# quan-dao/practical-collab-perception

Hardware: AMD Instinct MI355X
Metric: frames/sec (60k-pt cloud, 6 agents) (higher is better)
Workload: dtype f32

## Files before the change

practical-collab-perception_amd/csrc/sparseconv.hip:

```cpp
#include "pcp_common.h"

namespace {

constexpr int SP_TH = 8, SP_TW = 16, SP_PIX = SP_TH * SP_TW;
constexpr int SP_CIN = 64;
constexpr int SP_ALD = 68;
constexpr int SP_THREADS = 256;

struct SpParams {
  const float *pf;
  const int *cell_rank;
  const float *w;
  const float *bias;
  float *out;
  int batch, nx, ny, ho, wo, ld_out, cout, relu;
  int tiles_x, tiles_y;
};


template <bool OUT_BF16>
__global__ __launch_bounds__(SP_THREADS, 2) void k_sparse_conv_s2(SpParams p) {
  __shared__ __attribute__((aligned(16))) float acc[SP_PIX * 64];
#ifdef SP_ROW_SPLIT
  __shared__ __attribute__((aligned(16))) float atile[2][32 * SP_ALD];
#else
  __shared__ __attribute__((aligned(16))) float atile[4][32 * SP_ALD];
#endif
  __shared__ int row_rank[9][SP_PIX];
  __shared__ unsigned char row_pix[9][SP_PIX];
  __shared__ int cnt[9][2];

  const int tid = threadIdx.x, lane = tid & 63;
  const int wave = __builtin_amdgcn_readfirstlane(tid >> 6);
  int sp = blockIdx.x;
  const int tile_x = sp % p.tiles_x;
  sp /= p.tiles_x;
  const int tile_y = sp % p.tiles_y;
  const int b = sp / p.tiles_y;
  const int oy0 = tile_y * SP_TH, ox0 = tile_x * SP_TW;
  const int plane = p.nx * p.ny;

  int rank[9];
  {
    const int py = tid >> 4, px = tid & 15;
    const int oy = oy0 + py, ox = ox0 + px;
    const bool pix_ok = tid < SP_PIX && oy < p.ho && ox < p.wo;
#pragma unroll
    for (int t = 0; t < 9; t++) {
      const int iy = 2 * oy + t / 3 - 1, ix = 2 * ox + t % 3 - 1;
      rank[t] = -1;
      if (pix_ok && iy >= 0 && iy < p.ny && ix >= 0 && ix < p.nx) rank[t] = p.cell_rank[(long long)b * plane + ix * p.ny + iy];
    }
  }
  for (int i = tid; i < SP_PIX * 64; i += SP_THREADS) acc[i] = 0.f;
  int pre[9];
#pragma unroll
  for (int t = 0; t < 9; t++) {
    const unsigned long long bal = __ballot(rank[t] >= 0);
    pre[t] = __popcll(bal & ((1ULL << lane) - 1ULL));
    if (lane == 0 && wave < 2) cnt[t][wave] = __popcll(bal);
  }
  __syncthreads();
  int total = 0;
#pragma unroll
  for (int t = 0; t < 9; t++) {
    const int c0 = cnt[t][0], c1 = cnt[t][1];
    total += c0 + c1;
    if (tid < SP_PIX && rank[t] >= 0) {
      const int row = (wave == 1 ? c0 : 0) + pre[t];
      row_rank[t][row] = rank[t];
      row_pix[t][row] = (unsigned char)tid;
    }
  }
  __syncthreads();

#ifdef SP_ROW_SPLIT
  if (total > 0) {
    const int rh = wave >> 1, nh = wave & 1;
    const int m16 = lane & 15, q4 = lane >> 4;
    const int g_row = tid >> 3, g_q = (tid & 7) * 2;
    __shared__ unsigned char item_tap[36], item_chunk[36];
    __shared__ int n_items_s;
    if (tid == 0) {
      int k = 0;
      for (int t = 0; t < 9; t++)
        for (int c0 = 0; c0 < cnt[t][0] + cnt[t][1]; c0 += 32) { item_tap[k] = (unsigned char)t; item_chunk[k] = (unsigned char)(c0 >> 5); k++; }
      n_items_s = k;
    }
    __syncthreads();
    const int n_items = n_items_s;
    constexpr int DEPTH = 4;
    f32x4 g[DEPTH][2];
    f32x4 wq[2][2][4];
    auto gather = [&](int k, f32x4 (&dst)[2]) {
      const int kc = min(k, n_items - 1);
      const int t = item_tap[kc], c0 = item_chunk[kc] * 32;
      const int row = min(c0 + g_row, cnt[t][0] + cnt[t][1] - 1);
      const float *src = p.pf + (long long)row_rank[t][row] * SP_CIN + g_q * 4;
      dst[0] = *reinterpret_cast<const f32x4 *>(src);
      dst[1] = *reinterpret_cast<const f32x4 *>(src + 4);
    };
    auto wload = [&](int k, f32x4 (&dst)[2][4]) {
      const int t = item_tap[min(k, n_items - 1)];
#pragma unroll
      for (int s2 = 0; s2 < 2; s2++) {
        const float *wr = p.w + ((long long)(t * 64 + nh * 32 + s2 * 16 + m16)) * SP_CIN + 4 * q4;
#pragma unroll
        for (int j = 0; j < 4; j++) dst[s2][j] = *reinterpret_cast<const f32x4 *>(wr + 16 * j);
      }
    };
    wload(0, wq[0]);
    __builtin_amdgcn_sched_barrier(0);
    wload(1, wq[1]);
    __builtin_amdgcn_sched_barrier(0);
#pragma unroll
    for (int u = 0; u < DEPTH; u++) {
      gather(u, g[u]);
      __builtin_amdgcn_sched_barrier(0);
    }
    auto stage = [&](int k, f32x4 (&gu)[2], f32x4 (&wu)[2][4], float *at) {
          const int t = item_tap[k], c0 = item_chunk[k] * 32;
      const int rows = min(32, cnt[t][0] + cnt[t][1] - c0);
      const bool live = g_row < rows;
      const f32x4 zero4 = f32x4{0.f, 0.f, 0.f, 0.f};
      *reinterpret_cast<f32x4 *>(at + g_row * SP_ALD + g_q * 4) = live ? gu[0] : zero4;
      *reinterpret_cast<f32x4 *>(at + g_row * SP_ALD + g_q * 4 + 4) = live ? gu[1] : zero4;
      __builtin_amdgcn_sched_barrier(0);
      gather(k + DEPTH, gu);
      __builtin_amdgcn_sched_barrier(0);
      const unsigned pix4 = *reinterpret_cast<const unsigned *>(&row_pix[t][min(c0 + rh * 16 + q4 * 4, SP_PIX - 4)]);
      __syncthreads();
      typedef float f32x4c __attribute__((ext_vector_type(4)));
      f32x4c c0v = {0.f, 0.f, 0.f, 0.f}, c1v = {0.f, 0.f, 0.f, 0.f};
      const float *xa = at + (rh * 16 + m16) * SP_ALD + 4 * q4;
      f32x4 a[4];
#pragma unroll
      for (int j = 0; j < 4; j++) a[j] = *reinterpret_cast<const f32x4 *>(xa + 16 * j);
      int pixs[4];
      float old0[4], old1[4];
      const int col = nh * 32 + m16;
#pragma unroll
      for (int i = 0; i < 4; i++) {
        const int row = rh * 16 + q4 * 4 + i;
        pixs[i] = row < rows ? (int)((pix4 >> (8 * i)) & 255u) : -1;
        const int pa = pixs[i] >= 0 ? pixs[i] : 0;
        old0[i] = acc[pa * 64 + col];
        old1[i] = acc[pa * 64 + col + 16];
      }
#pragma unroll
      for (int j = 0; j < 4; j++)
#pragma unroll
        for (int kk = 0; kk < 4; kk++) {
          c0v = __builtin_amdgcn_mfma_f32_16x16x4f32(a[j][kk], wu[0][j][kk], c0v, 0, 0, 0);
          c1v = __builtin_amdgcn_mfma_f32_16x16x4f32(a[j][kk], wu[1][j][kk], c1v, 0, 0, 0);
        }
      __builtin_amdgcn_sched_barrier(0);
      wload(k + 2, wu);
      __builtin_amdgcn_sched_barrier(0);
#pragma unroll
      for (int i = 0; i < 4; i++)
        if (pixs[i] >= 0) {
          acc[pixs[i] * 64 + col] = old0[i] + c0v[i];
          acc[pixs[i] * 64 + col + 16] = old1[i] + c1v[i];
        }
    };
    int k0 = 0;
    for (; k0 + DEPTH <= n_items; k0 += DEPTH) {
      stage(k0 + 0, g[0], wq[0], atile[0]);
      stage(k0 + 1, g[1], wq[1], atile[1]);
      stage(k0 + 2, g[2], wq[0], atile[0]);
      stage(k0 + 3, g[3], wq[1], atile[1]);
    }
    if (k0 + 0 < n_items) stage(k0 + 0, g[0], wq[0], atile[0]);
    if (k0 + 1 < n_items) stage(k0 + 1, g[1], wq[1], atile[1]);
    if (k0 + 2 < n_items) stage(k0 + 2, g[2], wq[0], atile[0]);
    __syncthreads();
  }

#else
  if (total > 0) {
    const int m16 = lane & 15, q4 = lane >> 4;
    const int g_row = tid >> 3, g_q = (tid & 7) * 2;
    __shared__ unsigned char item_tap[36], item_chunk[36];
    __shared__ int n_items_s;
    if (tid == 0) {
      int k = 0;
      for (int t = 0; t < 9; t++)
        for (int c0 = 0; c0 < cnt[t][0] + cnt[t][1]; c0 += 32) { item_tap[k] = (unsigned char)t; item_chunk[k] = (unsigned char)(c0 >> 5); k++; }
      n_items_s = k;
    }
    __syncthreads();
    const int n_items = n_items_s;
    f32x4 g[4][2];
    f32x4 wq[4][4];
    auto gather = [&](int k, f32x4 (&dst)[2]) {
      const int kc = min(k, n_items - 1);
      const int t = item_tap[kc], c0 = item_chunk[kc] * 32;
      const int row = min(c0 + g_row, cnt[t][0] + cnt[t][1] - 1);
      const float *src = p.pf + (long long)row_rank[t][row] * SP_CIN + g_q * 4;
      dst[0] = *reinterpret_cast<const f32x4 *>(src);
      dst[1] = *reinterpret_cast<const f32x4 *>(src + 4);
    };
    auto wload = [&](int k, f32x4 (&dst)[4]) {
      const int t = item_tap[min(k, n_items - 1)];
      const float *wr = p.w + ((long long)(t * 64 + wave * 16 + m16)) * SP_CIN + 4 * q4;
#pragma unroll
      for (int j = 0; j < 4; j++) dst[j] = *reinterpret_cast<const f32x4 *>(wr + 16 * j);
    };
#pragma unroll
    for (int u = 0; u < 4; u++) {
      wload(u, wq[u]);
      gather(u, g[u]);
      __builtin_amdgcn_sched_barrier(0);
    }
    typedef float f32x4c __attribute__((ext_vector_type(4)));
    const int col = wave * 16 + m16;
    auto stage = [&](int k, f32x4 (&g0)[2], f32x4 (&g1)[2], f32x4 (&w0)[4], f32x4 (&w1)[4], float *at0, float *at1) {
      const f32x4 zero4 = f32x4{0.f, 0.f, 0.f, 0.f};
      int rows_i[2], tap_i[2], c0_i[2];
#pragma unroll
      for (int it = 0; it < 2; it++) {
        const int kk = min(k + it, n_items - 1);
        tap_i[it] = item_tap[kk];
        c0_i[it] = item_chunk[kk] * 32;
        rows_i[it] = (k + it < n_items) ? min(32, cnt[tap_i[it]][0] + cnt[tap_i[it]][1] - c0_i[it]) : 0;
      }
      *reinterpret_cast<f32x4 *>(at0 + g_row * SP_ALD + g_q * 4) = g_row < rows_i[0] ? g0[0] : zero4;
      *reinterpret_cast<f32x4 *>(at0 + g_row * SP_ALD + g_q * 4 + 4) = g_row < rows_i[0] ? g0[1] : zero4;
      *reinterpret_cast<f32x4 *>(at1 + g_row * SP_ALD + g_q * 4) = g_row < rows_i[1] ? g1[0] : zero4;
      *reinterpret_cast<f32x4 *>(at1 + g_row * SP_ALD + g_q * 4 + 4) = g_row < rows_i[1] ? g1[1] : zero4;
      __builtin_amdgcn_sched_barrier(0);
      gather(k + 4, g0);
      gather(k + 5, g1);
      __builtin_amdgcn_sched_barrier(0);
      unsigned pix4[2][2];
#pragma unroll
      for (int it = 0; it < 2; it++)
#pragma unroll
        for (int rtile = 0; rtile < 2; rtile++)
          pix4[it][rtile] = *reinterpret_cast<const unsigned *>(&row_pix[tap_i[it]][min(c0_i[it] + rtile * 16 + q4 * 4, SP_PIX - 4)]);
      __syncthreads();
      int pixs[2][2][4];
      float old0[2][4];
#pragma unroll
      for (int it = 0; it < 2; it++)
#pragma unroll
        for (int rtile = 0; rtile < 2; rtile++)
#pragma unroll
          for (int i = 0; i < 4; i++)
            pixs[it][rtile][i] = (rtile * 16 + q4 * 4 + i < rows_i[it]) ? (int)((pix4[it][rtile] >> (8 * i)) & 255u) : -1;
#pragma unroll
      for (int rtile = 0; rtile < 2; rtile++)
#pragma unroll
        for (int i = 0; i < 4; i++) old0[rtile][i] = acc[max(pixs[0][rtile][i], 0) * 64 + col];
      f32x4c cv[2][2];
#pragma unroll
      for (int it = 0; it < 2; it++) {
        const float *at = it == 0 ? at0 : at1;
#pragma unroll
        for (int rtile = 0; rtile < 2; rtile++) {
          f32x4c c = {0.f, 0.f, 0.f, 0.f};
          if (rows_i[it] > 16 * rtile) {
            f32x4 a[4];
#pragma unroll
            for (int j = 0; j < 4; j++) a[j] = *reinterpret_cast<const f32x4 *>(at + (rtile * 16 + m16) * SP_ALD + 16 * j + 4 * q4);
#pragma unroll
            for (int j = 0; j < 4; j++)
#pragma unroll
              for (int kk = 0; kk < 4; kk++) c = __builtin_amdgcn_mfma_f32_16x16x4f32(a[j][kk], (it == 0 ? w0 : w1)[j][kk], c, 0, 0, 0);
          }
          cv[it][rtile] = c;
        }
      }
      __builtin_amdgcn_sched_barrier(0);
      wload(k + 4, w0);
      wload(k + 5, w1);
      __builtin_amdgcn_sched_barrier(0);
#pragma unroll
      for (int rtile = 0; rtile < 2; rtile++)
#pragma unroll
        for (int i = 0; i < 4; i++)
          if (pixs[0][rtile][i] >= 0) acc[pixs[0][rtile][i] * 64 + col] = old0[rtile][i] + cv[0][rtile][i];
      float old1[2][4];
#pragma unroll
      for (int rtile = 0; rtile < 2; rtile++)
#pragma unroll
        for (int i = 0; i < 4; i++) old1[rtile][i] = acc[max(pixs[1][rtile][i], 0) * 64 + col];
#pragma unroll
      for (int rtile = 0; rtile < 2; rtile++)
#pragma unroll
        for (int i = 0; i < 4; i++)
          if (pixs[1][rtile][i] >= 0) acc[pixs[1][rtile][i] * 64 + col] = old1[rtile][i] + cv[1][rtile][i];
    };
    int k0 = 0;
    for (; k0 + 4 <= n_items; k0 += 4) {
      stage(k0 + 0, g[0], g[1], wq[0], wq[1], atile[0], atile[1]);
      stage(k0 + 2, g[2], g[3], wq[2], wq[3], atile[2], atile[3]);
    }
    if (k0 + 0 < n_items) stage(k0 + 0, g[0], g[1], wq[0], wq[1], atile[0], atile[1]);
    if (k0 + 2 < n_items) stage(k0 + 2, g[2], g[3], wq[2], wq[3], atile[2], atile[3]);
    __syncthreads();
  }
#endif

  {
    const int n4 = (tid & 15) * 4;
    const f32x4 bv = *reinterpret_cast<const f32x4 *>(p.bias + n4);
#pragma unroll
    for (int i = 0; i < 8; i++) {
      const int pix = (tid >> 4) + 16 * i;
      const int oy = oy0 + (pix >> 4), ox = ox0 + (pix & 15);
      if (oy < p.ho && ox < p.wo && n4 < p.cout) {
        f32x4 v = *reinterpret_cast<const f32x4 *>(acc + pix * 64 + n4) + bv;
        if (p.relu) {
          v.x = fmaxf(v.x, 0.f);
          v.y = fmaxf(v.y, 0.f);
          v.z = fmaxf(v.z, 0.f);
          v.w = fmaxf(v.w, 0.f);
        }
        const long long o = ((long long)(b * p.ho + oy) * p.wo + ox) * p.ld_out + n4;
        if (OUT_BF16) {
          typedef __bf16 b4 __attribute__((ext_vector_type(4)));
          b4 q;
          q[0] = (__bf16)v.x; q[1] = (__bf16)v.y; q[2] = (__bf16)v.z; q[3] = (__bf16)v.w;
          *reinterpret_cast<b4 *>(reinterpret_cast<__bf16 *>(p.out) + o) = q;
        } else {
          *reinterpret_cast<f32x4 *>(p.out + o) = v;
        }
      }
    }
  }
}

}

static int sparse_conv_impl(const float *pillar_features, const pcp_grid_t *grid, const void *vox_workspace, int64_t n, const float *w_packed,
                            const float *bias, int32_t cout, int32_t relu, void *out, int out_bf16, int32_t ld_out, void *stream_) {
  if (!pillar_features || !grid || !vox_workspace || !w_packed || !bias || !out || n < 0) return PCP_ERR_ARG;
  if (cout <= 0 || cout > 64 || cout % 4 != 0 || ld_out % 4 != 0 || ld_out < cout) return PCP_ERR_UNSUPPORTED;
  if ((((uintptr_t)pillar_features) & 15) || (((uintptr_t)w_packed) & 15) || (((uintptr_t)bias) & 15) || (((uintptr_t)out) & (out_bf16 ? 7 : 15)))
    return PCP_ERR_ARG;
  if (grid->batch_size <= 0 || grid->nx <= 0 || grid->ny <= 0) return PCP_ERR_ARG;
  const int64_t cells = (int64_t)grid->batch_size * grid->nx * grid->ny;
  VoxLayout L = pcp_vox_layout(cells, n);
  SpParams p;
  p.pf = pillar_features;
  p.cell_rank = reinterpret_cast<const int *>(reinterpret_cast<const char *>(vox_workspace) + L.cell_rank);
  p.w = w_packed; p.bias = bias; p.out = (float *)out;
  p.batch = grid->batch_size; p.nx = grid->nx; p.ny = grid->ny;
  p.ho = (grid->ny - 1) / 2 + 1;
  p.wo = (grid->nx - 1) / 2 + 1;
  p.ld_out = ld_out; p.cout = cout; p.relu = relu;
  p.tiles_x = (p.wo + SP_TW - 1) / SP_TW;
  p.tiles_y = (p.ho + SP_TH - 1) / SP_TH;
  const long long blocks = (long long)p.batch * p.tiles_x * p.tiles_y;
  if (blocks > 0x7fffffffLL) return PCP_ERR_ARG;
  if (out_bf16) hipLaunchKernelGGL(k_sparse_conv_s2<true>, dim3((unsigned)blocks), dim3(SP_THREADS), 0, (hipStream_t)stream_, p);
  else hipLaunchKernelGGL(k_sparse_conv_s2<false>, dim3((unsigned)blocks), dim3(SP_THREADS), 0, (hipStream_t)stream_, p);
  PCP_CHECK_LAUNCH();
  return PCP_OK;
}

extern "C" int pcp_sparse_conv3x3_s2(const float *pillar_features, const pcp_grid_t *grid, const void *vox_workspace, int64_t n,
                                     const float *w_packed, const float *bias, int32_t cout, int32_t relu, float *out, int32_t ld_out,
                                     void *stream_) {
  return sparse_conv_impl(pillar_features, grid, vox_workspace, n, w_packed, bias, cout, relu, out, 0, ld_out, stream_);
}

extern "C" int pcp_mp_sparse_conv3x3_s2(const float *pillar_features, const pcp_grid_t *grid, const void *vox_workspace, int64_t n,
                                        const float *w_packed, const float *bias, int32_t cout, int32_t relu, void *out, int32_t out_dtype,
                                        int32_t ld_out, void *stream_) {
  if (out_dtype != 0 && out_dtype != 1) return PCP_ERR_ARG;
  return sparse_conv_impl(pillar_features, grid, vox_workspace, n, w_packed, bias, cout, relu, out, out_dtype, ld_out, stream_);
}
```

Before: 398.7.

## Make sparse conv kernel persistent with cross-tile prefetch of ranks and features

Turns the sparse 3x3 stride-2 conv into a persistent kernel: the grid is capped at two blocks per CU, and each block walks a strided, rotated sequence of tiles. The next tile's cell ranks are loaded while the current tile computes. Compaction and priming of gathers and weights for the next tile are issued before the current tile's epilogue. The epilogue zeroes the accumulator as it reads it, so no separate clear pass is needed per tile. The unused SP_ROW_SPLIT path is removed. The aim is to hide per-block launch and setup latency and overlap global loads across tiles. The cost is more complex control flow and less parallelism when the tile count is small or uneven across blocks.

New measurement: 398.2, median of 2. No clear change (-0.1%).

```diff
diff --git a/practical-collab-perception_amd/csrc/sparseconv.hip b/practical-collab-perception_amd/csrc/sparseconv.hip
--- a/practical-collab-perception_amd/csrc/sparseconv.hip
+++ b/practical-collab-perception_amd/csrc/sparseconv.hip
@@ -14,304 +14,189 @@
   const float *bias;
   float *out;
   int batch, nx, ny, ho, wo, ld_out, cout, relu;
-  int tiles_x, tiles_y;
+  int tiles_x, tiles_y, n_tiles;
 };
 
 
 template <bool OUT_BF16>
 __global__ __launch_bounds__(SP_THREADS, 2) void k_sparse_conv_s2(SpParams p) {
   __shared__ __attribute__((aligned(16))) float acc[SP_PIX * 64];
-#ifdef SP_ROW_SPLIT
-  __shared__ __attribute__((aligned(16))) float atile[2][32 * SP_ALD];
-#else
   __shared__ __attribute__((aligned(16))) float atile[4][32 * SP_ALD];
-#endif
   __shared__ int row_rank[9][SP_PIX];
   __shared__ unsigned char row_pix[9][SP_PIX];
   __shared__ int cnt[9][2];
+  __shared__ unsigned char item_tap[36], item_chunk[36];
 
   const int tid = threadIdx.x, lane = tid & 63;
   const int wave = __builtin_amdgcn_readfirstlane(tid >> 6);
-  int sp = blockIdx.x;
-  const int tile_x = sp % p.tiles_x;
-  sp /= p.tiles_x;
-  const int tile_y = sp % p.tiles_y;
-  const int b = sp / p.tiles_y;
-  const int oy0 = tile_y * SP_TH, ox0 = tile_x * SP_TW;
   const int plane = p.nx * p.ny;
-
-  int rank[9];
-  {
-    const int py = tid >> 4, px = tid & 15;
-    const int oy = oy0 + py, ox = ox0 + px;
-    const bool pix_ok = tid < SP_PIX && oy < p.ho && ox < p.wo;
+  const unsigned grid = gridDim.x;
+  auto tile_of = [&](int i) -> int {
+    const long long id = (long long)i * grid + (blockIdx.x + 37u * (unsigned)i) % grid;
+    return id < p.n_tiles ? (int)id : -1;
+  };
+
+  auto load_ranks = [&](int sp, int (&rk)[9], unsigned &ok) {
+    const int spc = max(sp, 0);
+    const int tile_x = spc % p.tiles_x, r = spc / p.tiles_x;
+    const int tile_y = r % p.tiles_y, b = r / p.tiles_y;
+    const int oy = tile_y * SP_TH + ((tid >> 4) & (SP_TH - 1)), ox = tile_x * SP_TW + (tid & 15);
+    const bool pix_ok = sp >= 0 && tid < SP_PIX && oy < p.ho && ox < p.wo;
+    const int *base = p.cell_rank + (long long)b * plane;
+    ok = 0;
 #pragma unroll
     for (int t = 0; t < 9; t++) {
       const int iy = 2 * oy + t / 3 - 1, ix = 2 * ox + t % 3 - 1;
-      rank[t] = -1;
-      if (pix_ok && iy >= 0 && iy < p.ny && ix >= 0 && ix < p.nx) rank[t] = p.cell_rank[(long long)b * plane + ix * p.ny + iy];
-    }
-  }
-  for (int i = tid; i < SP_PIX * 64; i += SP_THREADS) acc[i] = 0.f;
-  int pre[9];
-#pragma unroll
-  for (int t = 0; t < 9; t++) {
-    const unsigned long long bal = __ballot(rank[t] >= 0);
-    pre[t] = __popcll(bal & ((1ULL << lane) - 1ULL));
-    if (lane == 0 && wave < 2) cnt[t][wave] = __popcll(bal);
-  }
-  __syncthreads();
-  int total = 0;
-#pragma unroll
-  for (int t = 0; t < 9; t++) {
-    const int c0 = cnt[t][0], c1 = cnt[t][1];
-    total += c0 + c1;
-    if (tid < SP_PIX && rank[t] >= 0) {
-      const int row = (wave == 1 ? c0 : 0) + pre[t];
-      row_rank[t][row] = rank[t];
-      row_pix[t][row] = (unsigned char)tid;
-    }
-  }
-  __syncthreads();
-
-#ifdef SP_ROW_SPLIT
-  if (total > 0) {
-    const int rh = wave >> 1, nh = wave & 1;
-    const int m16 = lane & 15, q4 = lane >> 4;
-    const int g_row = tid >> 3, g_q = (tid & 7) * 2;
-    __shared__ unsigned char item_tap[36], item_chunk[36];
-    __shared__ int n_items_s;
-    if (tid == 0) {
-      int k = 0;
-      for (int t = 0; t < 9; t++)
-        for (int c0 = 0; c0 < cnt[t][0] + cnt[t][1]; c0 += 32) { item_tap[k] = (unsigned char)t; item_chunk[k] = (unsigned char)(c0 >> 5); k++; }
-      n_items_s = k;
-    }
-    __syncthreads();
-    const int n_items = n_items_s;
-    constexpr int DEPTH = 4;
-    f32x4 g[DEPTH][2];
-    f32x4 wq[2][2][4];
-    auto gather = [&](int k, f32x4 (&dst)[2]) {
-      const int kc = min(k, n_items - 1);
-      const int t = item_tap[kc], c0 = item_chunk[kc] * 32;
-      const int row = min(c0 + g_row, cnt[t][0] + cnt[t][1] - 1);
-      const float *src = p.pf + (long long)row_rank[t][row] * SP_CIN + g_q * 4;
-      dst[0] = *reinterpret_cast<const f32x4 *>(src);
-      dst[1] = *reinterpret_cast<const f32x4 *>(src + 4);
-    };
-    auto wload = [&](int k, f32x4 (&dst)[2][4]) {
-      const int t = item_tap[min(k, n_items - 1)];
-#pragma unroll
-      for (int s2 = 0; s2 < 2; s2++) {
-        const float *wr = p.w + ((long long)(t * 64 + nh * 32 + s2 * 16 + m16)) * SP_CIN + 4 * q4;
-#pragma unroll
-        for (int j = 0; j < 4; j++) dst[s2][j] = *reinterpret_cast<const f32x4 *>(wr + 16 * j);
-      }
-    };
-    wload(0, wq[0]);
-    __builtin_amdgcn_sched_barrier(0);
-    wload(1, wq[1]);
-    __builtin_amdgcn_sched_barrier(0);
-#pragma unroll
-    for (int u = 0; u < DEPTH; u++) {
-      gather(u, g[u]);
-      __builtin_amdgcn_sched_barrier(0);
-    }
-    auto stage = [&](int k, f32x4 (&gu)[2], f32x4 (&wu)[2][4], float *at) {
-          const int t = item_tap[k], c0 = item_chunk[k] * 32;
-      const int rows = min(32, cnt[t][0] + cnt[t][1] - c0);
-      const bool live = g_row < rows;
-      const f32x4 zero4 = f32x4{0.f, 0.f, 0.f, 0.f};
-      *reinterpret_cast<f32x4 *>(at + g_row * SP_ALD + g_q * 4) = live ? gu[0] : zero4;
-      *reinterpret_cast<f32x4 *>(at + g_row * SP_ALD + g_q * 4 + 4) = live ? gu[1] : zero4;
-      __builtin_amdgcn_sched_barrier(0);
-      gather(k + DEPTH, gu);
-      __builtin_amdgcn_sched_barrier(0);
-      const unsigned pix4 = *reinterpret_cast<const unsigned *>(&row_pix[t][min(c0 + rh * 16 + q4 * 4, SP_PIX - 4)]);
-      __syncthreads();
-      typedef float f32x4c __attribute__((ext_vector_type(4)));
-      f32x4c c0v = {0.f, 0.f, 0.f, 0.f}, c1v = {0.f, 0.f, 0.f, 0.f};
-      const float *xa = at + (rh * 16 + m16) * SP_ALD + 4 * q4;
-      f32x4 a[4];
-#pragma unroll
-      for (int j = 0; j < 4; j++) a[j] = *reinterpret_cast<const f32x4 *>(xa + 16 * j);
-      int pixs[4];
-      float old0[4], old1[4];
-      const int col = nh * 32 + m16;
-#pragma unroll
-      for (int i = 0; i < 4; i++) {
-        const int row = rh * 16 + q4 * 4 + i;
-        pixs[i] = row < rows ? (int)((pix4 >> (8 * i)) & 255u) : -1;
-        const int pa = pixs[i] >= 0 ? pixs[i] : 0;
-        old0[i] = acc[pa * 64 + col];
-        old1[i] = acc[pa * 64 + col + 16];
-      }
-#pragma unroll
-      for (int j = 0; j < 4; j++)
-#pragma unroll
-        for (int kk = 0; kk < 4; kk++) {
-          c0v = __builtin_amdgcn_mfma_f32_16x16x4f32(a[j][kk], wu[0][j][kk], c0v, 0, 0, 0);
-          c1v = __builtin_amdgcn_mfma_f32_16x16x4f32(a[j][kk], wu[1][j][kk], c1v, 0, 0, 0);
-        }
-      __builtin_amdgcn_sched_barrier(0);
-      wload(k + 2, wu);
-      __builtin_amdgcn_sched_barrier(0);
-#pragma unroll
-      for (int i = 0; i < 4; i++)
-        if (pixs[i] >= 0) {
-          acc[pixs[i] * 64 + col] = old0[i] + c0v[i];
-          acc[pixs[i] * 64 + col + 16] = old1[i] + c1v[i];
-        }
-    };
-    int k0 = 0;
-    for (; k0 + DEPTH <= n_items; k0 += DEPTH) {
-      stage(k0 + 0, g[0], wq[0], atile[0]);
-      stage(k0 + 1, g[1], wq[1], atile[1]);
-      stage(k0 + 2, g[2], wq[0], atile[0]);
-      stage(k0 + 3, g[3], wq[1], atile[1]);
-    }
-    if (k0 + 0 < n_items) stage(k0 + 0, g[0], wq[0], atile[0]);
-    if (k0 + 1 < n_items) stage(k0 + 1, g[1], wq[1], atile[1]);
-    if (k0 + 2 < n_items) stage(k0 + 2, g[2], wq[0], atile[0]);
-    __syncthreads();
-  }
-
-#else
-  if (total > 0) {
-    const int m16 = lane & 15, q4 = lane >> 4;
-    const int g_row = tid >> 3, g_q = (tid & 7) * 2;
-    __shared__ unsigned char item_tap[36], item_chunk[36];
-    __shared__ int n_items_s;
-    if (tid == 0) {
-      int k = 0;
-      for (int t = 0; t < 9; t++)
-        for (int c0 = 0; c0 < cnt[t][0] + cnt[t][1]; c0 += 32) { item_tap[k] = (unsigned char)t; item_chunk[k] = (unsigned char)(c0 >> 5); k++; }
-      n_items_s = k;
-    }
-    __syncthreads();
-    const int n_items = n_items_s;
-    f32x4 g[4][2];
-    f32x4 wq[4][4];
-    auto gather = [&](int k, f32x4 (&dst)[2]) {
-      const int kc = min(k, n_items - 1);
-      const int t = item_tap[kc], c0 = item_chunk[kc] * 32;
-      const int row = min(c0 + g_row, cnt[t][0] + cnt[t][1] - 1);
-      const float *src = p.pf + (long long)row_rank[t][row] * SP_CIN + g_q * 4;
-      dst[0] = *reinterpret_cast<const f32x4 *>(src);
-      dst[1] = *reinterpret_cast<const f32x4 *>(src + 4);
-    };
-    auto wload = [&](int k, f32x4 (&dst)[4]) {
-      const int t = item_tap[min(k, n_items - 1)];
-      const float *wr = p.w + ((long long)(t * 64 + wave * 16 + m16)) * SP_CIN + 4 * q4;
-#pragma unroll
-      for (int j = 0; j < 4; j++) dst[j] = *reinterpret_cast<const f32x4 *>(wr + 16 * j);
-    };
+      const bool in = pix_ok && iy >= 0 && iy < p.ny && ix >= 0 && ix < p.nx;
+      ok |= in ? 1u << t : 0u;
+      rk[t] = base[min(max(ix, 0), p.nx - 1) * p.ny + min(max(iy, 0), p.ny - 1)];
+    }
+  };
+  auto compact = [&](const int (&rk)[9], unsigned ok) -> int {
+    int rank[9], pre[9];
+#pragma unroll
+    for (int t = 0; t < 9; t++) {
+      rank[t] = ((ok >> t) & 1u) ? rk[t] : -1;
+      const unsigned long long bal = __ballot(rank[t] >= 0);
+      pre[t] = __popcll(bal & ((1ULL << lane) - 1ULL));
+      if (lane == 0 && wave < 2) cnt[t][wave] = __popcll(bal);
+    }
+    __syncthreads();
+    int n = 0;
+#pragma unroll
+    for (int t = 0; t < 9; t++) {
+      const int c0 = cnt[t][0], c1 = cnt[t][1];
+      if (tid < SP_PIX && rank[t] >= 0) {
+        const int row = (wave == 1 ? c0 : 0) + pre[t];
+        row_rank[t][row] = rank[t];
+        row_pix[t][row] = (unsigned char)tid;
+      }
+      const int n_t = (c0 + c1 + 31) >> 5, ch = tid - n;
+      if (ch >= 0 && ch < n_t) { item_tap[tid] = (unsigned char)t; item_chunk[tid] = (unsigned char)ch; }
+      n += n_t;
+    }
+    __syncthreads();
+    return __builtin_amdgcn_readfirstlane(n);
+  };
+
+  const int m16 = lane & 15, q4 = lane >> 4;
+  const int g_row = tid >> 3, g_q = (tid & 7) * 2;
+  const int col = wave * 16 + m16;
+  int n_items = 0;
+  f32x4 g[4][2];
+  f32x4 wq[4][4];
+  auto gather = [&](int k, f32x4 (&dst)[2]) {
+    const int kc = min(k, n_items - 1);
+    const int t = item_tap[kc], c0 = item_chunk[kc] * 32;
+    const int row = min(c0 + g_row, cnt[t][0] + cnt[t][1] - 1);
+    const float *src = p.pf + (long long)row_rank[t][row] * SP_CIN + g_q * 4;
+    dst[0] = *reinterpret_cast<const f32x4 *>(src);
+    dst[1] = *reinterpret_cast<const f32x4 *>(src + 4);
+  };
+  auto wload = [&](int k, f32x4 (&dst)[4]) {
+    const int t = item_tap[min(k, n_items - 1)];
+    const float *wr = p.w + ((long long)(t * 64 + wave * 16 + m16)) * SP_CIN + 4 * q4;
+#pragma unroll
+    for (int j = 0; j < 4; j++) dst[j] = *reinterpret_cast<const f32x4 *>(wr + 16 * j);
+  };
+  auto prime = [&]() {
 #pragma unroll
     for (int u = 0; u < 4; u++) {
       wload(u, wq[u]);
       gather(u, g[u]);
       __builtin_amdgcn_sched_barrier(0);
     }
-    typedef float f32x4c __attribute__((ext_vector_type(4)));
-    const int col = wave * 16 + m16;
-    auto stage = [&](int k, f32x4 (&g0)[2], f32x4 (&g1)[2], f32x4 (&w0)[4], f32x4 (&w1)[4], float *at0, float *at1) {
-      const f32x4 zero4 = f32x4{0.f, 0.f, 0.f, 0.f};
-      int rows_i[2], tap_i[2], c0_i[2];
-#pragma unroll
-      for (int it = 0; it < 2; it++) {
-        const int kk = min(k + it, n_items - 1);
-        tap_i[it] = item_tap[kk];
-        c0_i[it] = item_chunk[kk] * 32;
-        rows_i[it] = (k + it < n_items) ? min(32, cnt[tap_i[it]][0] + cnt[tap_i[it]][1] - c0_i[it]) : 0;
-      }
-      *reinterpret_cast<f32x4 *>(at0 + g_row * SP_ALD + g_q * 4) = g_row < rows_i[0] ? g0[0] : zero4;
-      *reinterpret_cast<f32x4 *>(at0 + g_row * SP_ALD + g_q * 4 + 4) = g_row < rows_i[0] ? g0[1] : zero4;
-      *reinterpret_cast<f32x4 *>(at1 + g_row * SP_ALD + g_q * 4) = g_row < rows_i[1] ? g1[0] : zero4;
-      *reinterpret_cast<f32x4 *>(at1 + g_row * SP_ALD + g_q * 4 + 4) = g_row < rows_i[1] ? g1[1] : zero4;
-      __builtin_amdgcn_sched_barrier(0);
-      gather(k + 4, g0);
-      gather(k + 5, g1);
-      __builtin_amdgcn_sched_barrier(0);
-      unsigned pix4[2][2];
-#pragma unroll
-      for (int it = 0; it < 2; it++)
-#pragma unroll
-        for (int rtile = 0; rtile < 2; rtile++)
-          pix4[it][rtile] = *reinterpret_cast<const unsigned *>(&row_pix[tap_i[it]][min(c0_i[it] + rtile * 16 + q4 * 4, SP_PIX - 4)]);
-      __syncthreads();
-      int pixs[2][2][4];
-      float old0[2][4];
-#pragma unroll
-      for (int it = 0; it < 2; it++)
-#pragma unroll
-        for (int rtile = 0; rtile < 2; rtile++)
-#pragma unroll
-          for (int i = 0; i < 4; i++)
-            pixs[it][rtile][i] = (rtile * 16 + q4 * 4 + i < rows_i[it]) ? (int)((pix4[it][rtile] >> (8 * i)) & 255u) : -1;
+  };
+  typedef float f32x4c __attribute__((ext_vector_type(4)));
+  auto stage = [&](int k, f32x4 (&g0)[2], f32x4 (&g1)[2], f32x4 (&w0)[4], f32x4 (&w1)[4], float *at0, float *at1) {
+    const f32x4 zero4 = f32x4{0.f, 0.f, 0.f, 0.f};
+    int rows_i[2], tap_i[2], c0_i[2];
+#pragma unroll
+    for (int it = 0; it < 2; it++) {
+      const int kk = min(k + it, n_items - 1);
+      tap_i[it] = item_tap[kk];
+      c0_i[it] = item_chunk[kk] * 32;
+      rows_i[it] = (k + it < n_items) ? min(32, cnt[tap_i[it]][0] + cnt[tap_i[it]][1] - c0_i[it]) : 0;
+    }
+    *reinterpret_cast<f32x4 *>(at0 + g_row * SP_ALD + g_q * 4) = g_row < rows_i[0] ? g0[0] : zero4;
+    *reinterpret_cast<f32x4 *>(at0 + g_row * SP_ALD + g_q * 4 + 4) = g_row < rows_i[0] ? g0[1] : zero4;
+    *reinterpret_cast<f32x4 *>(at1 + g_row * SP_ALD + g_q * 4) = g_row < rows_i[1] ? g1[0] : zero4;
+    *reinterpret_cast<f32x4 *>(at1 + g_row * SP_ALD + g_q * 4 + 4) = g_row < rows_i[1] ? g1[1] : zero4;
+    __builtin_amdgcn_sched_barrier(0);
+    gather(k + 4, g0);
+    gather(k + 5, g1);
+    __builtin_amdgcn_sched_barrier(0);
+    unsigned pix4[2][2];
+#pragma unroll
+    for (int it = 0; it < 2; it++)
 #pragma unroll
       for (int rtile = 0; rtile < 2; rtile++)
-#pragma unroll
-        for (int i = 0; i < 4; i++) old0[rtile][i] = acc[max(pixs[0][rtile][i], 0) * 64 + col];
-      f32x4c cv[2][2];
-#pragma unroll
-      for (int it = 0; it < 2; it++) {
-        const float *at = it == 0 ? at0 : at1;
-#pragma unroll
-        for (int rtile = 0; rtile < 2; rtile++) {
-          f32x4c c = {0.f, 0.f, 0.f, 0.f};
-          if (rows_i[it] > 16 * rtile) {
-            f32x4 a[4];
-#pragma unroll
-            for (int j = 0; j < 4; j++) a[j] = *reinterpret_cast<const f32x4 *>(at + (rtile * 16 + m16) * SP_ALD + 16 * j + 4 * q4);
-#pragma unroll
-            for (int j = 0; j < 4; j++)
-#pragma unroll
-              for (int kk = 0; kk < 4; kk++) c = __builtin_amdgcn_mfma_f32_16x16x4f32(a[j][kk], (it == 0 ? w0 : w1)[j][kk], c, 0, 0, 0);
-          }
-          cv[it][rtile] = c;
+        pix4[it][rtile] = *reinterpret_cast<const unsigned *>(&row_pix[tap_i[it]][min(c0_i[it] + rtile * 16 + q4 * 4, SP_PIX - 4)]);
+    __syncthreads();
+    int pixs[2][2][4];
+    float old0[2][4];
+#pragma unroll
+    for (int it = 0; it < 2; it++)
+#pragma unroll
+      for (int rtile = 0; rtile < 2; rtile++)
+#pragma unroll
+        for (int i = 0; i < 4; i++)
+          pixs[it][rtile][i] = (rtile * 16 + q4 * 4 + i < rows_i[it]) ? (int)((pix4[it][rtile] >> (8 * i)) & 255u) : -1;
+#pragma unroll
+    for (int rtile = 0; rtile < 2; rtile++)
+#pragma unroll
+      for (int i = 0; i < 4; i++) old0[rtile][i] = acc[max(pixs[0][rtile][i], 0) * 64 + col];
+    f32x4c cv[2][2];
+#pragma unroll
+    for (int it = 0; it < 2; it++) {
+      const float *at = it == 0 ? at0 : at1;
+#pragma unroll
+      for (int rtile = 0; rtile < 2; rtile++) {
+        f32x4c c = {0.f, 0.f, 0.f, 0.f};
+        if (rows_i[it] > 16 * rtile) {
+          f32x4 a[4];
+#pragma unroll
+          for (int j = 0; j < 4; j++) a[j] = *reinterpret_cast<const f32x4 *>(at + (rtile * 16 + m16) * SP_ALD + 16 * j + 4 * q4);
+#pragma unroll
+          for (int j = 0; j < 4; j++)
+#pragma unroll
+            for (int kk = 0; kk < 4; kk++) c = __builtin_amdgcn_mfma_f32_16x16x4f32(a[j][kk], (it == 0 ? w0 : w1)[j][kk], c, 0, 0, 0);
         }
-      }
-      __builtin_amdgcn_sched_barrier(0);
-      wload(k + 4, w0);
-      wload(k + 5, w1);
-      __builtin_amdgcn_sched_barrier(0);
-#pragma unroll
-      for (int rtile = 0; rtile < 2; rtile++)
-#pragma unroll
-        for (int i = 0; i < 4; i++)
-          if (pixs[0][rtile][i] >= 0) acc[pixs[0][rtile][i] * 64 + col] = old0[rtile][i] + cv[0][rtile][i];
-      float old1[2][4];
-#pragma unroll
-      for (int rtile = 0; rtile < 2; rtile++)
-#pragma unroll
-        for (int i = 0; i < 4; i++) old1[rtile][i] = acc[max(pixs[1][rtile][i], 0) * 64 + col];
-#pragma unroll
-      for (int rtile = 0; rtile < 2; rtile++)
-#pragma unroll
-        for (int i = 0; i < 4; i++)
-          if (pixs[1][rtile][i] >= 0) acc[pixs[1][rtile][i] * 64 + col] = old1[rtile][i] + cv[1][rtile][i];
-    };
-    int k0 = 0;
-    for (; k0 + 4 <= n_items; k0 += 4) {
-      stage(k0 + 0, g[0], g[1], wq[0], wq[1], atile[0], atile[1]);
-      stage(k0 + 2, g[2], g[3], wq[2], wq[3], atile[2], atile[3]);
-    }
-    if (k0 + 0 < n_items) stage(k0 + 0, g[0], g[1], wq[0], wq[1], atile[0], atile[1]);
-    if (k0 + 2 < n_items) stage(k0 + 2, g[2], g[3], wq[2], wq[3], atile[2], atile[3]);
-    __syncthreads();
-  }
-#endif
-
-  {
-    const int n4 = (tid & 15) * 4;
-    const f32x4 bv = *reinterpret_cast<const f32x4 *>(p.bias + n4);
+        cv[it][rtile] = c;
+      }
+    }
+    __builtin_amdgcn_sched_barrier(0);
+    wload(k + 4, w0);
+    wload(k + 5, w1);
+    __builtin_amdgcn_sched_barrier(0);
+#pragma unroll
+    for (int rtile = 0; rtile < 2; rtile++)
+#pragma unroll
+      for (int i = 0; i < 4; i++)
+        if (pixs[0][rtile][i] >= 0) acc[pixs[0][rtile][i] * 64 + col] = old0[rtile][i] + cv[0][rtile][i];
+    float old1[2][4];
+#pragma unroll
+    for (int rtile = 0; rtile < 2; rtile++)
+#pragma unroll
+      for (int i = 0; i < 4; i++) old1[rtile][i] = acc[max(pixs[1][rtile][i], 0) * 64 + col];
+#pragma unroll
+    for (int rtile = 0; rtile < 2; rtile++)
+#pragma unroll
+      for (int i = 0; i < 4; i++)
+        if (pixs[1][rtile][i] >= 0) acc[pixs[1][rtile][i] * 64 + col] = old1[rtile][i] + cv[1][rtile][i];
+  };
+  const int n4 = (tid & 15) * 4;
+  const f32x4 bv = *reinterpret_cast<const f32x4 *>(p.bias + n4);
+  auto epilogue = [&](int sp) {
+    const int tile_x = sp % p.tiles_x, r = sp / p.tiles_x;
+    const int oy0 = (r % p.tiles_y) * SP_TH, ox0 = tile_x * SP_TW, b = r / p.tiles_y;
 #pragma unroll
     for (int i = 0; i < 8; i++) {
       const int pix = (tid >> 4) + 16 * i;
       const int oy = oy0 + (pix >> 4), ox = ox0 + (pix & 15);
+      f32x4 v = *reinterpret_cast<const f32x4 *>(acc + pix * 64 + n4) + bv;
+      *reinterpret_cast<f32x4 *>(acc + pix * 64 + n4) = f32x4{0.f, 0.f, 0.f, 0.f};
       if (oy < p.ho && ox < p.wo && n4 < p.cout) {
-        f32x4 v = *reinterpret_cast<const f32x4 *>(acc + pix * 64 + n4) + bv;
         if (p.relu) {
           v.x = fmaxf(v.x, 0.f);
           v.y = fmaxf(v.y, 0.f);
@@ -329,6 +214,37 @@
         }
       }
     }
+  };
+
+  int rk[9];
+  unsigned rk_ok;
+  int cur = tile_of(0);
+  load_ranks(cur, rk, rk_ok);
+  for (int i = tid; i < SP_PIX * 16; i += SP_THREADS) reinterpret_cast<f32x4 *>(acc)[i] = f32x4{0.f, 0.f, 0.f, 0.f};
+  n_items = compact(rk, rk_ok);
+  if (n_items > 0) prime();
+  int nxt = tile_of(1);
+  load_ranks(nxt, rk, rk_ok);
+  for (int round = 2;; round++) {
+    if (n_items > 0) {
+      int k0 = 0;
+      for (; k0 + 4 <= n_items; k0 += 4) {
+        stage(k0 + 0, g[0], g[1], wq[0], wq[1], atile[0], atile[1]);
+        stage(k0 + 2, g[2], g[3], wq[2], wq[3], atile[2], atile[3]);
+      }
+      if (k0 + 0 < n_items) stage(k0 + 0, g[0], g[1], wq[0], wq[1], atile[0], atile[1]);
+      if (k0 + 2 < n_items) stage(k0 + 2, g[2], g[3], wq[2], wq[3], atile[2], atile[3]);
+    }
+    __syncthreads();
+    if (nxt >= 0) {
+      n_items = compact(rk, rk_ok);
+      if (n_items > 0) prime();
+      load_ranks(tile_of(round), rk, rk_ok);
+    }
+    epilogue(cur);
+    if (nxt < 0) break;
+    cur = nxt;
+    nxt = tile_of(round);
   }
 }
 
@@ -353,8 +269,10 @@
   p.ld_out = ld_out; p.cout = cout; p.relu = relu;
   p.tiles_x = (p.wo + SP_TW - 1) / SP_TW;
   p.tiles_y = (p.ho + SP_TH - 1) / SP_TH;
-  const long long blocks = (long long)p.batch * p.tiles_x * p.tiles_y;
-  if (blocks > 0x7fffffffLL) return PCP_ERR_ARG;
+  const long long tiles = (long long)p.batch * p.tiles_x * p.tiles_y;
+  if (tiles > 0x7fffffffLL) return PCP_ERR_ARG;
+  p.n_tiles = (int)tiles;
+  const long long blocks = std::min<long long>(tiles, 2LL * std::max(pcp_current_device_cus(), 1));
   if (out_bf16) hipLaunchKernelGGL(k_sparse_conv_s2<true>, dim3((unsigned)blocks), dim3(SP_THREADS), 0, (hipStream_t)stream_, p);
   else hipLaunchKernelGGL(k_sparse_conv_s2<false>, dim3((unsigned)blocks), dim3(SP_THREADS), 0, (hipStream_t)stream_, p);
   PCP_CHECK_LAUNCH();
```
